# ilovin/lstm_ctc_ocr

Hardware: AMD Instinct MI355X
Metric: captcha images/sec training (32x256, bs=64/GPU) (higher is better)
Workload: dtype bf16; 1 GPU; VGG-7 + BiLSTM(256) + CTC train step, H=32 W=256, 10-char labels, C=64, bs=64/GPU (BASELINE.json configs[1]), Adam lr 1e-4 wd 1e-5 clip 10; global_batch=64, parallelism=dp1, hipgraph=True

## Files before the change

include/ocr_hip.h:

```cpp
#ifndef OCR_HIP_H
#define OCR_HIP_H
#include <stddef.h>
#ifdef __cplusplus
extern "C" {
#endif

enum { OCR_STATUS_OK = 0, OCR_STATUS_MEMOPS = 1, OCR_STATUS_INVALID = 2, OCR_STATUS_EXEC = 3 };

enum {
    OCR_EPI_BIAS = 1, OCR_EPI_RELU = 2, OCR_EPI_OUT_F32 = 4,
    OCR_EPI_MASK = 16, OCR_EPI_ROWSWAP = 32, OCR_EPI_ACCUM = 64
};

const char* ocr_status_string(int status);
int ocr_abi_version(void);
const char* ocr_build_id(void);

int ocr_ctc_workspace_size(int max_label_len, int max_time, int minibatch, size_t* bytes);
int ocr_ctc_loss(const float* activations, float* gradients, const int* flat_labels, const int* label_lengths,
                 const int* input_lengths, int alphabet_size, int minibatch, int max_time, int max_label_len,
                 int blank_label, float* costs, void* workspace, void* stream);
int ocr_ctc_debug(void* dbg);
int ocr_ctc_train_supported(int alphabet_size, int max_time, int max_label_len);
int ocr_ctc_loss_train(const float* activations, void* grad_ntc_bf16, float scale, const int* flat_labels,
// ... 51 lines not shown
                             long strideColsum, void* stream);
typedef struct ocr_tn_job {
    const void* A; long lda; long strideA;
    const void* B; long ldb; long strideB;
    float* out; long ldo; long strideOut;
    float* colsum; long strideColsum;
    int Mk, I, J, nbatch;
    int row_group, row_skip;
    float scale; int reserved;
} ocr_tn_job;
int ocr_gemm_tn_jobs_supported(const ocr_tn_job* jobs, int njobs);
int ocr_gemm_tn_jobs_bf16(const ocr_tn_job* jobs, int njobs, void* stream);
int ocr_set_wgrad_engine(int engine);
int ocr_conv3x3_wgrad_bf16(const void* x, const void* dy, float* dw, float* dbias, int Nb, int W, int H, int Cin,
                           int Cout, int splits, void* stream);
int ocr_conv3x3_wgrad_kernel_choice(int Nb, int W, int H, int Cin, int Cout, int has_workspace, int splits);

int ocr_conv3x3_wgrad_workspace_size(int Nb, int W, int H, int Cin, int Cout, size_t* bytes);
int ocr_conv3x3_wgrad_ws_bf16(const void* x, const void* dy, float* dw, float* dbias, int Nb, int W, int H, int Cin,
                              int Cout, int splits, void* workspace, size_t workspace_bytes, void* stream);
int ocr_conv3x3_wgrad_defer_bf16(const void* x, const void* dy, float* dw, float* dbias, int Nb, int W, int H, int Cin, int Cout,
                                 void* workspace, size_t workspace_bytes, void* job, int* job_blocks, int* deferred, void* stream);
int ocr_wgrad9_reduce_jobs(const void* jobs, int njobs, int total_blocks, void* stream);
int ocr_conv3x3_wgrad_pair_supported(const int* shape_first, const int* shape_second);
int ocr_conv3x3_wgrad_pair_defer_bf16(const void* x0, const void* dy0, float* dw0, float* dbias0, const int* shape0, void* workspace0,
                                      size_t workspace_bytes0, const void* x1, const void* dy1, float* dw1, float* dbias1, const int* shape1,
                                      void* workspace1, size_t workspace_bytes1, void* job0, void* job1, int* job_blocks0, int* job_blocks1,
                                      void* stream);

int ocr_conv1_fwd(const float* x, const float* w, const float* bias, void* y, int Nb, int W, int H, int Cout,
                  int relu, void* stream);
int ocr_conv1_wgrad(const float* x, const void* dz, float* dw, float* db, int Nb, int W, int H, int Cout,
                    void* stream);
int ocr_eltwise_bf16(int op, const void* a, const void* b, void* out, long n, void* stream);
int ocr_conv1_pool_fwd(const float* x, const float* w, const float* bias, void* p, int Nb, int W, int H, int Cout, void* stream);
int ocr_conv1_pool_fwd_train(const float* x, const float* w, const float* bias, void* p, int Nb, int W, int H, int Cout,
                             void* codes, float* zero, long zero_n, void* ones, long ones_n, void* stream);
int ocr_conv1_pool_bwd_codes(const float* x, const float* w, const float* bias, const void* dp, float* dw, float* db,
                             int Nb, int W, int H, int Cout, const void* codes, void* stream);
int ocr_conv1_pool_bwd_slab_rows(int Nb, int W, int H);
int ocr_conv1_pool_bwd_slab(const float* x, const float* w, const float* bias, const void* dp, int Nb, int W, int H, int Cout,
                            const void* codes, float* slab, void* stream);
int ocr_conv1_pool_bwd(const float* x, const float* w, const float* bias, const void* dp, float* dw, float* db, int Nb,
                       int W, int H, int Cout, void* stream);
int ocr_maxpool_fwd(const void* x, void* y, int Nb, int W, int H, int C, int kw, int kh, void* stream);
int ocr_maxpool_bwd(const void* x, const void* dy, void* dx, int Nb, int W, int H, int C, int kw, int kh,
// ... 105 lines not shown
```

lstm_ctc_ocr_amd/_native.py:

```python
import ctypes
import os
import re

_HERE = os.path.dirname(os.path.abspath(__file__))
LIB_PATH = os.environ.get("OCR_NATIVE_LIB") or os.path.join(_HERE, "libocrhip.so")
HEADER_PATH = os.path.join(os.path.dirname(_HERE), "include", "ocr_hip.h")

EPI_BIAS, EPI_RELU, EPI_OUT_F32, EPI_MASK, EPI_ROWSWAP, EPI_ACCUM = 1, 2, 4, 16, 32, 64

_P, _I, _L, _F, _D = ctypes.c_void_p, ctypes.c_int, ctypes.c_long, ctypes.c_float, ctypes.c_double

_SIGS = {
    "ocr_abi_version": ([], _I),
    "ocr_build_id": ([], ctypes.c_char_p),
    "ocr_status_string": ([_I], ctypes.c_char_p),
    "ocr_ctc_workspace_size": ([_I, _I, _I, ctypes.POINTER(ctypes.c_size_t)], _I),
    "ocr_ctc_loss": ([_P, _P, _P, _P, _P, _I, _I, _I, _I, _I, _P, _P, _P], _I),
    "ocr_set_ctc_engine": ([_I], _I),
    "ocr_ctc_debug": ([_P], _I),
    "ocr_ctc_train_supported": ([_I, _I, _I], _I),
    "ocr_ctc_loss_train": ([_P, _P, _F, _P, _P, _P, _I, _I, _I, _I, _I, _P, _P], _I),
    "ocr_ctc_long_placement": ([_I, _I, _I], _I),
    "ocr_ctc_long_supported": ([_I, _I, _I], _I),
    "ocr_ctc_long_workspace_size": ([_I, _I, _I, _I, ctypes.POINTER(ctypes.c_size_t)], _I),
    "ocr_ctc_loss_long": ([_P, _P, _P, _F, _P, _P, _P, _I, _I, _I, _I, _I, _P, _P, ctypes.c_size_t, _P], _I),
    "ocr_ctc_greedy_decode": ([_P, _P, _I, _I, _I, _I, _I, _P, _P, _P], _I),
    "ocr_ctc_beam_workspace_size": ([_I, _I, _I, _I, ctypes.POINTER(ctypes.c_size_t)], _I),
    "ocr_ctc_beam_decode": ([_P, _P, _I, _I, _I, _I, _I, _I, _P, _P, _P, _P, ctypes.c_size_t, _P], _I),
    "ocr_ctc_beam_kernel_choice": ([_I, _I], _I),
    "ocr_set_beam_engine": ([_I], _I),
    "ocr_gemm_nt_bf16": ([_P, _L, _P, _L, _P, _L, _I, _I, _I, _P, _P, _L, _I, _I, _I, _I, _I, _I, _P], _I),
    "ocr_set_gemm_engine": ([_I], _I),
    "ocr_gemm_tn_batched_bf16": ([_P, _L, _L, _P, _L, _L, _P, _L, _L, _I, _I, _I, _I, _F, _I, _P, _L, _P], _I),
    "ocr_gemm_tn_jobs_supported": ([_P, _I], _I),
    "ocr_gemm_tn_jobs_bf16": ([_P, _I, _P], _I),
    "ocr_lstm_xh": ([_P, _P, _P, _P, _I, _I, _I, _I, _I, _P], _I),
    "ocr_set_wgrad_engine": ([_I], _I),
    "ocr_conv3x3_bf16": ([_P, _P, _P, _I, _I, _I, _I, _I, _P, _P, _I, _P], _I),
    "ocr_conv_halo_clock_debug": ([_P], _I),
    "ocr_occupy_cus": ([_I, _I, _I, _F, _P], _I),
    "ocr_conv_ws_debug": ([_P], _I),
    "ocr_conv3x3_accum_supported": ([_I, _I, _I, _I, _I], _I),
    "ocr_conv3x3_kernel_choice": ([_I, _I, _I, _I, _I, _I, _I, _I], _I),
    "ocr_conv3x3_pool_supported": ([_I, _I, _I, _I, _I, _I, _I], _I),
    "ocr_conv3x3_relu_pool_bf16": ([_P, _P, _P, _P, _I, _I, _I, _I, _I, _P, _I, _I, _P], _I),
    "ocr_conv3x3_pool_codes_supported": ([_I, _I, _I, _I, _I, _I, _I], _I),
    "ocr_conv3x3_relu_pool_codes_bf16": ([_P, _P, _P, _P, _P, _I, _I, _I, _I, _I, _P, _I, _I, _P], _I),
    "ocr_gemm_tn_bf16": ([_P, _L, _P, _L, _P, _L, _I, _I, _I, _I, _I, _L, _F, _I, _P, _P], _I),
    "ocr_gemm_tn_split_workspace_floats": ([_I, _I, _I], _L),
    "ocr_gemm_tn_split_bf16": ([_P, _L, _P, _L, _P, _L, _I, _I, _I, _F, _P, _P, _L, _P], _I),
    "ocr_conv3x3_wgrad_bf16": ([_P, _P, _P, _P, _I, _I, _I, _I, _I, _I, _P], _I),
    "ocr_conv3x3_wgrad_kernel_choice": ([_I, _I, _I, _I, _I, _I, _I], _I),
    "ocr_conv3x3_wgrad_workspace_size": ([_I, _I, _I, _I, _I, ctypes.POINTER(ctypes.c_size_t)], _I),
    "ocr_conv3x3_wgrad_ws_bf16": ([_P, _P, _P, _P, _I, _I, _I, _I, _I, _I, _P, ctypes.c_size_t, _P], _I),
    "ocr_conv3x3_wgrad_defer_bf16": ([_P, _P, _P, _P, _I, _I, _I, _I, _I, _P, ctypes.c_size_t, _P, ctypes.POINTER(_I),
                                      ctypes.POINTER(_I), _P], _I),
    "ocr_conv3x3_wgrad_pair_supported": ([ctypes.POINTER(_I), ctypes.POINTER(_I)], _I),
    "ocr_conv3x3_wgrad_pair_defer_bf16": ([_P, _P, _P, _P, ctypes.POINTER(_I), _P, ctypes.c_size_t, _P, _P, _P, _P, ctypes.POINTER(_I), _P,
# ... 68 lines not shown
    "ocr_probe_tr16": ([_P, _P, _P], _I),
    "ocr_set_lstm_proto": ([_I], _I),
    "ocr_set_lstm_ksplit": ([_I], _I),
    "ocr_probe_xcc": ([_P, _I, _I, _P], _I),
    "ocr_mfma_busy_probe": ([_P, _I, _I, _I, _P, _P], _I),
}


class NativeError(RuntimeError):
    pass


def declared_symbols(header=HEADER_PATH):
    text = open(header).read()
    text = re.sub(r"/\*.*?\*/", "", text, flags=re.S)
    return sorted(set(re.findall(r"\b(ocr_[a-z0-9_]+)\s*\(", text)))


def source_build_id(csrc=os.path.join(_HERE, "csrc"), experiments=False):
    import glob
    import hashlib
    rel = [os.path.basename(f) for f in glob.glob(os.path.join(csrc, "*.hip"))]
    h = hashlib.sha256()
    for f in sorted(rel) + ["common.h", "conv_plan.h", "Makefile"]:
        h.update(open(os.path.join(csrc, f), "rb").read())
    return h.hexdigest()[:16] + ("-exp" if experiments else "")


def build_id():
    return lib().ocr_build_id().decode()


_lib = None


def lib():
    global _lib
    if _lib is None:
        if not os.path.exists(LIB_PATH):
            raise NativeError(
                "libocrhip.so not found at %s — build it with `python -c 'import __graft_entry__ as g; g.build()'` "
                "(there is no CPU/eager fallback for the hot path)" % LIB_PATH)
        _lib = ctypes.CDLL(LIB_PATH)
        for name, (argtypes, restype) in _SIGS.items():
            fn = getattr(_lib, name)
            fn.argtypes = argtypes
            fn.restype = restype
# ... 24 lines not shown
```

lstm_ctc_ocr_amd/csrc/gemm_tn3.hip:

```cpp
#include "common.h"
#include <stdlib.h>
#include <type_traits>

struct Tn3Job {
    const bf16_t* A; long lda; long sA;
    const bf16_t* B; long ldb; long sB;
    float* out; long ldo; long sO;
    float* colsum; long sC;
    int Mk, I, J, nbatch;
    int grp, skip;
    float scale; int reserved;
};
static_assert(sizeof(Tn3Job) == 120, "mirrored by lstm_ctc_ocr_amd/ops.py (ctypes.Structure)");

__device__ u32x4 tn3_zero_page[4];

typedef const __attribute__((address_space(1))) void* gptr_t;
typedef __attribute__((address_space(3))) void* lptr_t;
typedef __attribute__((ext_vector_type(4))) short s16x4;
typedef __attribute__((ext_vector_type(8))) short s16x8;

__device__ __forceinline__ int tn3_frag_off(int cb, int lane) {
    const int g = lane >> 4, L = lane & 15;
    const int r0 = 4 * g + (L >> 2);
// ... 186 lines not shown
                old[a2][b][r] = __builtin_nontemporal_load(out + (long)(i0 + wi * 64 + (KH * 2 + a2) * 16 + (lane >> 4) * 4 + r) * g.ldo + j0 + wj * 64 + b * 16 + (lane & 15));
#pragma unroll
    for (int a2 = 0; a2 < 2; ++a2)
#pragma unroll
        for (int b = 0; b < 4; ++b)
#pragma unroll
            for (int r = 0; r < 4; ++r)
                out[(long)(i0 + wi * 64 + (KH * 2 + a2) * 16 + (lane >> 4) * 4 + r) * g.ldo + j0 + wj * 64 + b * 16 + (lane & 15)] =
                    old[a2][b][r] + acc[KH * 2 + a2][b][r] * scale;
}

template <int NST>
__global__ __launch_bounds__(512) __attribute__((amdgpu_waves_per_eu(2, 2))) void gemm_tn3_kernel(Tn3Job j0, Tn3Job j1, int nblk0) {
    extern __shared__ __attribute__((aligned(16))) unsigned char smem[];
    const int kh = __builtin_amdgcn_readfirstlane((int)(threadIdx.x >> 8));
    const int bid = (int)blockIdx.x;
    if (bid < nblk0) {
        if (kh == 0) tn3_body<0, NST>(j0, bid, smem); else tn3_body<1, NST>(j0, bid, smem);
    } else {
        if (kh == 0) tn3_body<0, NST>(j1, bid - nblk0, smem); else tn3_body<1, NST>(j1, bid - nblk0, smem);
    }
}

static bool tn3_covers(const Tn3Job& j) {
    if (!j.A || !j.B || !j.out || j.Mk < 256 || j.I <= 0 || j.J <= 0 || (j.I & 127) || (j.J & 127) || j.nbatch < 1) return false;
    if ((j.lda & 7) || (j.ldb & 7) || (j.sA & 7) || (j.sB & 7) || ((size_t)j.A & 15) || ((size_t)j.B & 15)) return false;
    if (j.grp < 0 || j.skip < 0 || (j.grp == 0 && j.skip != 0)) return false;
    return (long)(j.I >> 7) * (j.J >> 7) * j.nbatch <= 0x7fffffL;
}
extern "C" int ocr_gemm_tn_jobs_supported(const void* jobs, int njobs) {
    if (!jobs || njobs < 1 || njobs > 2) return 0;
    const Tn3Job* j = (const Tn3Job*)jobs;
    for (int k = 0; k < njobs; ++k) if (!tn3_covers(j[k])) return 0;
    return 1;
}
extern "C" int ocr_gemm_tn_jobs_bf16(const void* jobs, int njobs, void* stream) {
    if (!ocr_gemm_tn_jobs_supported(jobs, njobs)) return OCR_ERR_INVALID;
    const Tn3Job* j = (const Tn3Job*)jobs;
    const int t0 = (j[0].I >> 7) * (j[0].J >> 7) * j[0].nbatch;
    const int t1 = njobs > 1 ? (j[1].I >> 7) * (j[1].J >> 7) * j[1].nbatch : 0;
    static int nst = -1;
    if (nst < 0) { const char* e = getenv("OCR_TN3_NST"); nst = (e && atoi(e) == 5) ? 5 : 4; }
    const int lds = nst * 2 * 64 * 256;
    if (nst == 4) {
        if (ocr_allow_lds<gemm_tn3_kernel<4>>(lds) != hipSuccess) return OCR_ERR_EXEC;
        gemm_tn3_kernel<4><<<t0 + t1, 512, lds, (hipStream_t)stream>>>(j[0], njobs > 1 ? j[1] : j[0], t0);
    } else {
        if (ocr_allow_lds<gemm_tn3_kernel<5>>(lds) != hipSuccess) return OCR_ERR_EXEC;
        gemm_tn3_kernel<5><<<t0 + t1, 512, lds, (hipStream_t)stream>>>(j[0], njobs > 1 ? j[1] : j[0], t0);
    }
    OCR_CHECK_LAUNCH();
    return OCR_OK;
}
```

lstm_ctc_ocr_amd/csrc/wgrad9.hip:

```cpp
#include "common.h"
#include <stdlib.h>
#include <utility>
#include <type_traits>

struct W9Args {
    const bf16_t* X; const bf16_t* dY;
    int M, Cin, Cout, cW, cH;
    int k_per_split;
    int S, T_ci, T_co, map;
    float* part;
    float* cs_part;
};

__device__ u32x4 w9_zero_page[4];
typedef const __attribute__((address_space(1))) void* gptr_t;
typedef __attribute__((address_space(3))) void* lptr_t;
typedef __attribute__((ext_vector_type(4))) short s16x4;

constexpr int W9_NDMA = 5;
constexpr int W9_STAGE = 8 * W9_NDMA * 1024;
constexpr int W9_NST = 3;
constexpr int W9_LA = 2;
constexpr int W9_NSLOT = W9_LA + 1;
constexpr int W9_DMA_AT = 3;
// ... 417 lines not shown
    __syncthreads();
    W9P_PHASE(1);

    if (do_cs) w9_cs_store(g, smem, cs, split, co0, tid);
    W9P_PHASE(2);
    w9_store_tile(g, smem, acc, split, ci0, co0, cb, kh, lane);
#ifdef OCR_EXPERIMENTS
    W9P_PHASE(3);
    asm volatile("s_waitcnt vmcnt(0)" ::: "memory");
    W9P_PHASE(4);
#endif
}
template <int H, bool GENW>
__global__ __launch_bounds__(512) void wgrad9p_kernel(W9Args g) { wgrad9p_body<H, GENW>(g, blockIdx.x); }

template <int H, bool GENW>
__global__ __launch_bounds__(512) void wgrad9p_kernel(W9Args first, W9Args second, int nblk_first) {
    const int b = blockIdx.x;
    if (b < nblk_first) wgrad9_body(first, b);
    else if constexpr (H == 16) wgrad9_body(second, b - nblk_first);
    else wgrad9p_body<H, GENW>(second, b - nblk_first);
}

__device__ __forceinline__ void w9_reduce_body(float* __restrict__ dw, const float* __restrict__ part, long n4, long slab4, int S, int rows,
                                               float* __restrict__ dbias, const float* __restrict__ cs_part, int Cout, int blk) {
    __shared__ f32x4 red[256];
    const int cols = 256 / rows;
    const int col = threadIdx.x % cols, row = threadIdx.x / cols;
    const long i = (long)blk * cols + col;
    f32x4 a = {0.f, 0.f, 0.f, 0.f}, t = a;
    if (i < n4) {
        f32x4 b = {0.f, 0.f, 0.f, 0.f}, c = b, d = b;
        const f32x4* p = (const f32x4*)part + i;
        if (row == 0) t = ((const f32x4*)dw)[i];
        int s = row;
        for (; s + 3 * rows < S; s += 4 * rows) {
            a += __builtin_nontemporal_load(p + (long)s * slab4);              b += __builtin_nontemporal_load(p + (long)(s + rows) * slab4);
            c += __builtin_nontemporal_load(p + (long)(s + 2 * rows) * slab4); d += __builtin_nontemporal_load(p + (long)(s + 3 * rows) * slab4);
        }
        for (; s < S; s += rows) a += __builtin_nontemporal_load(p + (long)s * slab4);
        a = (a + b) + (c + d);
    }
    red[row * cols + col] = a;
    __syncthreads();
    if (row == 0 && i < n4) {
        for (int r = 0; r < rows; ++r) t += red[r * cols + col];
        ((f32x4*)dw)[i] = t;
    }
    if (dbias != nullptr && blk == 0)
        for (int c = threadIdx.x; c < Cout; c += blockDim.x) {
            float t = dbias[c];
            for (int s = 0; s < S; ++s) t += cs_part[(long)s * Cout + c];
            dbias[c] = t;
        }
}
__global__ __launch_bounds__(256) void wgrad9_reduce_kernel(float* __restrict__ dw, const float* __restrict__ part, long n4, long slab4,
                                                            int S, int rows, float* __restrict__ dbias, const float* __restrict__ cs_part, int Cout) {
    w9_reduce_body(dw, part, n4, slab4, S, rows, dbias, cs_part, Cout, blockIdx.x);
}
struct W9ReduceJob {
    float* dw; const float* part; float* dbias; const float* cs_part;
    long n4, slab4;
    int S, rows, Cout, block_start;
};
__global__ __launch_bounds__(256) void wgrad9_reduce_jobs_kernel(const W9ReduceJob* __restrict__ jobs, int njobs) {
    __shared__ int jsel[4];
    int j = 0;
    for (int k = threadIdx.x; k < njobs; k += 256)
        if (jobs[k].block_start <= (int)blockIdx.x) j = k;
#pragma unroll
    for (int off = 32; off > 0; off >>= 1) j = max(j, __shfl_xor(j, off));
    if ((threadIdx.x & 63) == 0) jsel[threadIdx.x >> 6] = j;
    __syncthreads();
    j = max(max(jsel[0], jsel[1]), max(jsel[2], jsel[3]));
    const W9ReduceJob jb = jobs[j];
    w9_reduce_body(jb.dw, jb.part, jb.n4, jb.slab4, jb.S, jb.rows, jb.dbias, jb.cs_part, jb.Cout, (int)blockIdx.x - jb.block_start);
}

struct W9Plan { int S, k_per_split, map, T_ci, T_co; size_t bytes; };

static bool w9_plan(int M, int W, int H, int Cin, int Cout, W9Plan* p) {
    if ((Cin & 63) || (Cout & 63) || (H != 2 && H != 4 && H != 8 && H != 16) || M < 512 || (M % H) || W * H < 32) return false;
    const int T_ci = Cin / 64, T_co = Cout / 64, T = T_ci * T_co;
    static int smax = -1;
    if (smax < 0) { const char* e = ocr_tune_env("OCR_W9_SMAX"); smax = e ? atoi(e) : 64; if (smax < 1) smax = 1; }
    int S = 1;
    while ((long)S * 2 * T <= 256 && S * 2 <= smax && M / (S * 2) >= 512) S *= 2;
    p->S = S; p->T_ci = T_ci; p->T_co = T_co;
    p->k_per_split = ceil_div(ceil_div(M, S), 128) * 128;
    p->map = S >= 8 ? 1 : ((T % (8 / S)) == 0 ? 2 : 0);
    p->bytes = (size_t)S * ((size_t)9 * Cin * Cout + Cout) * sizeof(float);
    return true;
}

extern "C" int ocr_wgrad9_debug(void* dbg ) {
    long long* q = (long long*)dbg;
    return hipMemcpyToSymbol(HIP_SYMBOL(w9_dbg), &q, sizeof(q)) == hipSuccess ? OCR_OK : OCR_ERR_MEMOPS;
}

// ... 108 lines not shown
    if (!wgrad9_pair_ok(shape0[0], shape0[1], shape0[2], shape0[3], shape0[4], shape1[0], shape1[1], shape1[2], shape1[3], shape1[4])) return -1;
    W9Plan p0, p1;
    W9Args g0, g1;
    const int k0 = w9_setup(x[0], dy[0], dbias[0], shape0[0], shape0[1], shape0[2], shape0[3], shape0[4], workspace[0], ws_bytes[0], &p0, &g0);
    const int k1 = w9_setup(x[1], dy[1], dbias[1], shape1[0], shape1[1], shape1[2], shape1[3], shape1[4], workspace[1], ws_bytes[1], &p1, &g1);
    if (k0 != W9K_WGRAD9 || k1 < 0) return -1;
    const int grid0 = p0.S * p0.T_ci * p0.T_co, grid1 = p1.S * p1.T_ci * p1.T_co;
    int rc;
    switch (k1) {
        case W9K_P4: rc = w9_launch_pair<W9P_PAIR<4, false>>(g0, grid0, g1, grid1, stream); break;
        case W9K_P8: rc = w9_launch_pair<W9P_PAIR<8, false>>(g0, grid0, g1, grid1, stream); break;
        case W9K_P4_ZERO_ROW: rc = w9_launch_pair<W9P_PAIR<4, true>>(g0, grid0, g1, grid1, stream); break;
        case W9K_P8_ZERO_ROW: rc = w9_launch_pair<W9P_PAIR<8, true>>(g0, grid0, g1, grid1, stream); break;
        default: rc = w9_launch_pair<W9P_PAIR<16, false>>(g0, grid0, g1, grid1, stream); break;
    }
    if (rc != OCR_OK) return rc;
    OCR_CHECK_LAUNCH();
    *(W9ReduceJob*)job[0] = w9_reduce_job(g0, dw[0], dbias[0], job_blocks[0]);
    *(W9ReduceJob*)job[1] = w9_reduce_job(g1, dw[1], dbias[1], job_blocks[1]);
    return OCR_OK;
}

extern "C" int ocr_wgrad9_reduce_jobs(const void* jobs, int njobs, int total_blocks, void* stream) {
    static_assert(sizeof(W9ReduceJob) == 64, "W9ReduceJob is mirrored by engine.py");
    if (!jobs || njobs <= 0 || total_blocks <= 0) return OCR_ERR_INVALID;
    wgrad9_reduce_jobs_kernel<<<total_blocks, 256, 0, (hipStream_t)stream>>>((const W9ReduceJob*)jobs, njobs);
    OCR_CHECK_LAUNCH();
    return OCR_OK;
}
```

lstm_ctc_ocr_amd/engine.py:

```python
import time

import numpy as np
import torch

from . import dist as ocr_dist
from . import ops
from ._native import NativeError, call as nat_call
from .engine_ops import (BF16, F32, I32, _env, _number, _switch, _AddOp, _AvgPoolOp, _BatchNormOp, _BiLstmOp, _ConcatOp, _ConvOp,
                         _Conv3x3Op, _DropoutOp, _FcOp, _InputOp, _PoolOp, _ReluOp, _SoftmaxOp, _SubsampleOp, _ViewOp, _conv_op)
from .layout import FlatLayout, execution_order, init_host_parameters

ALIGN = 64





class ShapePlan(object):

    def _init_fields(self, N, W):
        self.N, self.W = N, W
        self.buf, self.shape = {}, {}
        self.scratch = {}
        self.dy_done = set()
        self.w9_pending, self.w9_tables = [], {}
        self.w9_pending_bytes = 0
        self.tn_pending = []
        self.w9_held = None
        self.tn_side_open = False
        self.fused_pools = set()
        self.bn_stat_rows = {}
        self.bn_bwd_rows = {}
        self.w9_hold_for = {}
        self.unpool_pools = set()
        self.col_bn = {}
        self.lstm_sync_keys = ()
        self.lstm_arena, self.lstm_sync = None, ()
        self.rings_ready, self.rings_armed = set(), False
        self.graph_fb = self.graph_fwd = self.graph_fb1 = self.graph_fb2 = self.graph_dp = self.graph_step = None
        self._guard_addrs = None
        self._report = None

    def __init__(self, eng, N, W):
        self._init_fields(N, W)
        dev = eng.device
        self.x = torch.zeros((N, W, eng.num_features), dtype=F32, device=dev)
        self.labels = torch.zeros(N * eng.max_label_len, dtype=I32, device=dev)
        self.labels_len = torch.zeros(N, dtype=I32, device=dev)
        self.seq_len = torch.ones(N, dtype=I32, device=dev)
        self.oshape = {'data': (N, W, eng.num_features)}
# ... 31 lines not shown
class Engine(object):

    def __init__(self, net, device='cuda:0', seed=None, max_label_len=31, use_graphs=True, group=None,
                 persistent_lstm=True, fuse_conv1_pool=True, ctc_long=True):
        from .config import cfg
        if max_label_len > self.CTC_MAX_LABEL_LEN:
            raise ValueError('max_label_len = %d: the CTC loss covers labels of at most %d characters' % (max_label_len, self.CTC_MAX_LABEL_LEN))
        if not torch.cuda.is_available():
            raise NativeError('Engine needs a ROCm GPU: the hot path has no CPU implementation')
        self.cfg = cfg
        self.net = net
        self.device = torch.device(device)
        torch.cuda.set_device(self.device)
        self.num_features = cfg.NUM_FEATURES
        self.max_label_len = max_label_len
        self.ctc_long = ctc_long
        self.use_graphs = use_graphs
        self.persistent_lstm = persistent_lstm
        self.fuse_conv1_pool = fuse_conv1_pool
        self.fuse_bn_stats = _switch('OCR_FUSE_BN_STATS')
        self.w9_flush_bytes = int(_number('OCR_W9_FLUSH_MB', 80, float) * (1 << 20))
        self.tn_defer = _switch('OCR_TN_JOBS')
        self.tn_side = _switch('OCR_TN_SIDE', False)
        self.side_stream = torch.cuda.Stream(device=self.device) if (self.tn_side and torch.device(self.device).type == 'cuda') else None
        self.group = group
        self.world = 1
        self._check_xcd_placement()
        self.force_allreduce = bool(_env('OCR_FORCE_ALLREDUCE'))
        if group is not None or (torch.distributed.is_available() and torch.distributed.is_initialized()):
            self.world = torch.distributed.get_world_size(group)
        if _env('OCR_FAKE_WORLD'):
            self.world = _number('OCR_FAKE_WORLD', None)
            self.force_allreduce = True
        self.overlap_allreduce = _switch('OCR_OVERLAP_ALLREDUCE')
        self.dp_graph = _env('OCR_DP_GRAPH', '0') == '1'
        self.defer_w9 = _switch('OCR_W9_DEFER')
        self.w9_pair = _switch('OCR_W9_PAIR')
        self.w9_defer_max_bytes = _number('OCR_W9_DEFER_MAX_MB', self.W9_DEFER_MAX_BYTES >> 20) << 20
        self.w9_ws_pool = {}
        self.comm_stream = torch.cuda.Stream(device=self.device)
        self.dp_host_s = [0.0, 0.0, 0.0, 0.0, 0.0, 0]
        self._pack_table = None
        self._fault_hook = None
        self._watch_pending = None
        self.dropped_reports = 0
        self._lower(net)
# ... 267 lines not shown
            d.copy_(t, non_blocking=True)

    def step_counter(self):
        return self.scalars[6:7]

    def _forward(self, sp, training=False):
        self.training = training
        self._zero_pending = bool(training) and self.grads.numel() % 4 == 0 and _switch('OCR_FUSE_ZERO')
        if training and not self._zero_pending:
            self.grads.zero_()
        sp.rings_ready, sp.rings_armed = set(), False
        self._ones_pending = sp.lstm_arena if (training and sp.lstm_arena is not None and _switch('OCR_FUSE_RINGFILL')) else None
        for op in self.ops:
            op.fwd(sp)
        self._ones_pending = None
        if self._zero_pending:
            self.grads.zero_()
            self._zero_pending = False

    def _loss_and_backward(self, sp, flush=True):
        sp.dy_done = set()
        sp.w9_pending = []
        sp.tn_pending = []
        sp.w9_held = None
        logits = self.ops[-1].y(sp)
        scale = ocr_dist.loss_scale(sp.N, self.world)
        path = self.ctc_path_of(sp.C, sp.T)
        if path == 'fast':
            ops.ctc_loss_train(logits, self.ops[-1].dy(sp), scale, sp.labels, sp.labels_len, sp.seq_len, self.max_label_len,
                               sp.costs, blank=0)
        elif path == 'long':
            ops.ctc_loss_long(logits, sp.labels, sp.labels_len, sp.seq_len, self.max_label_len, blank=0, want_grad=False,
                              grad_ntc_bf16=self.ops[-1].dy(sp), scale=scale, workspace=sp.ctc_ws, costs=sp.costs)
        else:
            ops.ctc_loss(logits, sp.labels, sp.labels_len, sp.seq_len, self.max_label_len, blank=0, want_grad=True,
                         workspace=sp.ctc_ws, costs=sp.costs, grads=sp.ctc_grad)
            ops.tnc_to_ntc_bf16(sp.ctc_grad, self.ops[-1].dy(sp), scale)
        for op in reversed(self.ops[self.split_op:]):
            op.bwd(sp)
        self._flush_tn(sp)
        self._join_tn(sp)
        self._release_w9(sp)
        if flush:
            self._flush_w9(sp)

    CTC_MAX_LABEL_LEN = 255

    def ctc_path_of(self, C, T):
        if ops.ctc_train_supported(C, T, self.max_label_len):
            return 'fast'
        if self.ctc_long and ops.ctc_long_supported(C, T, self.max_label_len):
            return 'long'
        return 'general'

    def ctc_path(self, N, W):
        sp = self.plan(N, W)
        return self.ctc_path_of(sp.C, sp.T)

    def _backward_early(self, sp):
        for op in reversed(self.ops[:self.split_op]):
            op.bwd(sp)
        self._flush_tn(sp)
        self._join_tn(sp)
        self._release_w9(sp)
        self._flush_w9(sp)

    def tn_push(self, sp, job, keep, fallback):
        if not self.tn_defer or not ops.gemm_tn_jobs_supported([job]):
            fallback()
            return
        sp.tn_pending.append((job, keep, fallback))
        if len(sp.tn_pending) == 2:
            self._flush_tn(sp)

    def _flush_tn(self, sp):
        pend, sp.tn_pending = sp.tn_pending, []
        if len(pend) == 2:
            if self.tn_side:
                main = torch.cuda.current_stream(self.device)
                self.side_stream.wait_stream(main)
                with torch.cuda.stream(self.side_stream):
                    ops.gemm_tn_jobs([pend[0][0], pend[1][0]])
                sp.tn_side_open = True
            else:
                ops.gemm_tn_jobs([pend[0][0], pend[1][0]])
        else:
            for _, _, fallback in pend:
                fallback()

    def _join_tn(self, sp):
        if sp.tn_side_open:
            torch.cuda.current_stream(self.device).wait_stream(self.side_stream)
            sp.tn_side_open = False

    W9_DEFER_MAX_BYTES = 192 << 20
    W9_JOB_DTYPE = np.dtype([('dw', '<u8'), ('part', '<u8'), ('dbias', '<u8'), ('cs_part', '<u8'), ('n4', '<i8'), ('slab4', '<i8'),
                             ('S', '<i4'), ('rows', '<i4'), ('Cout', '<i4'), ('block_start', '<i4')])

    def w9_append(self, sp, job, ws):
        sp.w9_pending.append(job)
        sp.w9_pending_bytes += ws.numel()
        if self.w9_flush_bytes and sp.w9_pending_bytes >= self.w9_flush_bytes:
            self._flush_w9(sp)

    def w9_hold(self, sp, key, x, dz, dw, db, ws):
        self._release_w9(sp)
        sp.w9_held = (key, x, dz, dw, db, ws)

    def _release_w9(self, sp):
        held, sp.w9_held = sp.w9_held, None
        if held is not None:
            _, x, dz, dw, db, ws = held
            job, nblk = ops.conv3x3_wgrad_deferred(x, dz, dw, db, ws)
            if job is not None:
                self.w9_append(sp, (job, nblk), ws)

    def _flush_w9(self, sp):
        self._release_w9(sp)
        pend, sp.w9_pending = sp.w9_pending, []
        sp.w9_pending_bytes = 0
        if not pend:
            return
        raw = b''.join(job for job, _ in pend)
        ent = sp.w9_tables.get(raw)
        if ent is None:
            tab = np.frombuffer(raw, dtype=self.W9_JOB_DTYPE).copy()
            assert tab.itemsize == 64 and len(tab) == len(pend)
            start = 0
            for i, (_, nblk) in enumerate(pend):
                tab['block_start'][i] = start
                start += nblk
            dev = torch.from_numpy(tab.view(np.uint8).copy()).to(self.device)
            ent = sp.w9_tables[raw] = (dev, len(pend), start)
        ops.wgrad9_reduce_jobs(*ent)

    def _capture(self, fn):
        import gc
        gc.collect()
        torch.cuda.synchronize()
        g = torch.cuda.CUDAGraph()
        was = gc.isenabled()
        gc.disable()
        try:
            with torch.cuda.graph(g, capture_error_mode='thread_local'):
                fn()
        finally:
            if was:
                gc.enable()
        return g

    def _run_split(self, sp):
        def body1():
            self._forward(sp, training=True)
            self._loss_and_backward(sp)
            self._publish_guard(sp)

        def body2():
# ... 319 lines not shown
```

lstm_ctc_ocr_amd/ops.py:

```python
import ctypes

import torch

from . import _native as nat
from ._native import EPI_ACCUM, EPI_BIAS, EPI_MASK, EPI_OUT_F32, EPI_RELU, EPI_ROWSWAP, call, ptr

BF16 = torch.bfloat16
F32 = torch.float32


def _st():
    return nat.stream()


def _dev(t):
    if not t.is_cuda:
        raise nat.NativeError("hot-path operators take device tensors only (got a CPU tensor)")
    return t


def ctc_workspace_bytes(max_label_len, max_time, minibatch):
    sz = ctypes.c_size_t(0)
    call("ocr_ctc_workspace_size", max_label_len, max_time, minibatch, ctypes.byref(sz))
    return sz.value
# ... 218 lines not shown
                ("B", ctypes.c_void_p), ("ldb", ctypes.c_long), ("strideB", ctypes.c_long),
                ("out", ctypes.c_void_p), ("ldo", ctypes.c_long), ("strideOut", ctypes.c_long),
                ("colsum", ctypes.c_void_p), ("strideColsum", ctypes.c_long),
                ("Mk", ctypes.c_int), ("I", ctypes.c_int), ("J", ctypes.c_int), ("nbatch", ctypes.c_int),
                ("row_group", ctypes.c_int), ("row_skip", ctypes.c_int), ("scale", ctypes.c_float), ("reserved", ctypes.c_int)]


def tn_job(A, lda, B, ldb, out, ldo, Mk, I, J, *, nbatch=1, strideA=0, strideB=0, strideOut=0, colsum=None, strideColsum=0, row_group=0,
           row_skip=0, scale=1.0):
    return TnJob(ptr(_dev(A)), lda, strideA, ptr(_dev(B)), ldb, strideB, ptr(out), ldo, strideOut, ptr(colsum), strideColsum,
                 Mk, I, J, nbatch, row_group, row_skip, float(scale), 0)


def gemm_tn_jobs_supported(jobs):
    arr = (TnJob * len(jobs))(*jobs)
    return bool(nat.lib().ocr_gemm_tn_jobs_supported(ctypes.cast(arr, ctypes.c_void_p), len(jobs)))


def gemm_tn_jobs(jobs):
    arr = (TnJob * len(jobs))(*jobs)
    call("ocr_gemm_tn_jobs_bf16", ctypes.cast(arr, ctypes.c_void_p), len(jobs), _st())


def lstm_xh(x2d, hout, seq_len, xh, Nb, T, D, U, ndir=2):
    call("ocr_lstm_xh", ptr(_dev(x2d)), ptr(hout), ptr(seq_len), ptr(xh), Nb, T, D, U, ndir, _st())
    return xh


def conv3x3_wgrad_workspace_bytes(Nb, W, H, Cin, Cout):
    sz = ctypes.c_size_t(0)
    call("ocr_conv3x3_wgrad_workspace_size", Nb, W, H, Cin, Cout, ctypes.byref(sz))
    return sz.value


WGRAD_KERNEL_NAMES = ("wgrad9", "wgrad9p<4>", "wgrad9p<8>", "wgrad9p<4>/zero-row", "wgrad9p<8>/zero-row", "gemm_tn2/nine-tap",
                      "gemm_tn2/paired-tap", "gemm_tn<1,4,4>", "gemm_tn<1,2,2>")


def conv3x3_wgrad_kernel_choice(Nb, W, H, Cin, Cout, *, workspace=True, splits=0):
    rc = nat.lib().ocr_conv3x3_wgrad_kernel_choice(int(Nb), int(W), int(H), int(Cin), int(Cout), int(bool(workspace)), int(splits))
    if rc < 0:
        raise nat.NativeError("ocr_conv3x3_wgrad_kernel_choice failed: status %d (%s)" % (-rc, nat.status_string(-rc)))
    return WGRAD_KERNEL_NAMES[rc & 255], rc >> 8


def conv3x3_wgrad(x, dy, dw, splits=0, dbias=None, workspace=None):
# ... 404 lines not shown
```

Baseline: 58120 images/sec.

## Fuse deferred TN weight-grad GEMM pair with wgrad9 split-K reduction launch

Holds the pending pair of TN weight-gradient GEMM jobs and, when the wgrad9 split-K reduce jobs are flushed, launches both in one kernel. The GEMM blocks come first and the tail blocks run the reduction as two virtual 256-thread blocks per 512-thread block, sharing LDS. This aims to remove one launch and the tail or idle gap between the GEMM and the small reduce kernel. The cost is that the reduce blocks now run at the GEMM kernel's LDS allocation and occupancy, and the held GEMM work may be delayed to the flush point, which changes the ordering.

```diff
diff --git a/include/ocr_hip.h b/include/ocr_hip.h
--- a/include/ocr_hip.h
+++ b/include/ocr_hip.h
@@ -97,6 +97,9 @@
 int ocr_conv3x3_wgrad_defer_bf16(const void* x, const void* dy, float* dw, float* dbias, int Nb, int W, int H, int Cin, int Cout,
                                  void* workspace, size_t workspace_bytes, void* job, int* job_blocks, int* deferred, void* stream);
 int ocr_wgrad9_reduce_jobs(const void* jobs, int njobs, int total_blocks, void* stream);
+int ocr_gemm_tn_jobs_reduce_supported(const ocr_tn_job* jobs, int njobs, const void* reduce_jobs, int n_reduce_jobs, int total_reduce_blocks);
+int ocr_gemm_tn_jobs_reduce_bf16(const ocr_tn_job* jobs, int njobs, const void* reduce_jobs, int n_reduce_jobs, int total_reduce_blocks,
+                                 void* stream);
 int ocr_conv3x3_wgrad_pair_supported(const int* shape_first, const int* shape_second);
 int ocr_conv3x3_wgrad_pair_defer_bf16(const void* x0, const void* dy0, float* dw0, float* dbias0, const int* shape0, void* workspace0,
                                       size_t workspace_bytes0, const void* x1, const void* dy1, float* dw1, float* dbias1, const int* shape1,
diff --git a/lstm_ctc_ocr_amd/_native.py b/lstm_ctc_ocr_amd/_native.py
--- a/lstm_ctc_ocr_amd/_native.py
+++ b/lstm_ctc_ocr_amd/_native.py
@@ -34,6 +34,8 @@
     "ocr_gemm_tn_batched_bf16": ([_P, _L, _L, _P, _L, _L, _P, _L, _L, _I, _I, _I, _I, _F, _I, _P, _L, _P], _I),
     "ocr_gemm_tn_jobs_supported": ([_P, _I], _I),
     "ocr_gemm_tn_jobs_bf16": ([_P, _I, _P], _I),
+    "ocr_gemm_tn_jobs_reduce_supported": ([_P, _I, _P, _I, _I], _I),
+    "ocr_gemm_tn_jobs_reduce_bf16": ([_P, _I, _P, _I, _I, _P], _I),
     "ocr_lstm_xh": ([_P, _P, _P, _P, _I, _I, _I, _I, _I, _P], _I),
     "ocr_set_wgrad_engine": ([_I], _I),
     "ocr_conv3x3_bf16": ([_P, _P, _P, _I, _I, _I, _I, _I, _P, _P, _I, _P], _I),
@@ -148,7 +150,7 @@
     import hashlib
     rel = [os.path.basename(f) for f in glob.glob(os.path.join(csrc, "*.hip"))]
     h = hashlib.sha256()
-    for f in sorted(rel) + ["common.h", "conv_plan.h", "Makefile"]:
+    for f in sorted(rel) + ["common.h", "conv_plan.h", "w9_reduce.h", "Makefile"]:
         h.update(open(os.path.join(csrc, f), "rb").read())
     return h.hexdigest()[:16] + ("-exp" if experiments else "")
 
diff --git a/lstm_ctc_ocr_amd/csrc/gemm_tn3.hip b/lstm_ctc_ocr_amd/csrc/gemm_tn3.hip
--- a/lstm_ctc_ocr_amd/csrc/gemm_tn3.hip
+++ b/lstm_ctc_ocr_amd/csrc/gemm_tn3.hip
@@ -1,4 +1,5 @@
 #include "common.h"
+#include "w9_reduce.h"
 #include <stdlib.h>
 #include <type_traits>
 
@@ -232,6 +233,26 @@
     }
 }
 
+template <int NST>
+__global__ __launch_bounds__(512) __attribute__((amdgpu_waves_per_eu(2, 2))) void gemm_tn3_kernel(Tn3Job j0, Tn3Job j1, int nblk0, int nblk_tn,
+                                                                                              const W9ReduceJob* __restrict__ jobs, int njobs, int nvirt) {
+    extern __shared__ __attribute__((aligned(16))) unsigned char smem[];
+    const int kh = __builtin_amdgcn_readfirstlane((int)(threadIdx.x >> 8));
+    const int bid = (int)blockIdx.x;
+    if (bid < nblk0) {
+        if (kh == 0) tn3_body<0, NST>(j0, bid, smem); else tn3_body<1, NST>(j0, bid, smem);
+    } else if (bid < nblk_tn) {
+        if (kh == 0) tn3_body<0, NST>(j1, bid - nblk0, smem); else tn3_body<1, NST>(j1, bid - nblk0, smem);
+    } else {
+        const int vblk = 2 * (bid - nblk_tn) + kh, tid = (int)threadIdx.x & (W9R_THREADS - 1);
+        f32x4* red = (f32x4*)(smem + kh * W9R_RED_BYTES);
+        int* jsel = (int*)(smem + 2 * W9R_RED_BYTES + kh * W9R_JSEL_BYTES);
+        const int j = w9_reduce_find_job(jobs, njobs, vblk, tid, jsel);
+        const W9ReduceJob jb = jobs[j];
+        w9_reduce_body(jb.dw, jb.part, jb.n4, jb.slab4, jb.S, jb.rows, jb.dbias, jb.cs_part, jb.Cout, vblk - jb.block_start, tid, red, vblk < nvirt);
+    }
+}
+
 static bool tn3_covers(const Tn3Job& j) {
     if (!j.A || !j.B || !j.out || j.Mk < 256 || j.I <= 0 || j.J <= 0 || (j.I & 127) || (j.J & 127) || j.nbatch < 1) return false;
     if ((j.lda & 7) || (j.ldb & 7) || (j.sA & 7) || (j.sB & 7) || ((size_t)j.A & 15) || ((size_t)j.B & 15)) return false;
@@ -244,21 +265,60 @@
     for (int k = 0; k < njobs; ++k) if (!tn3_covers(j[k])) return 0;
     return 1;
 }
+typedef void (*Tn3Kernel)(Tn3Job, Tn3Job, int);
+typedef void (*Tn3ReduceKernel)(Tn3Job, Tn3Job, int, int, const W9ReduceJob*, int, int);
+template <int NST> constexpr Tn3Kernel TN3_PLAIN = gemm_tn3_kernel<NST>;
+template <int NST> constexpr Tn3ReduceKernel TN3_REDUCE = gemm_tn3_kernel<NST>;
+
+static int tn3_stages() {
+    static int nst = -1;
+    if (nst < 0) { const char* e = getenv("OCR_TN3_NST"); nst = (e && atoi(e) == 5) ? 5 : 4; }
+    return nst;
+}
+static int tn3_tiles(const Tn3Job& j) { return (j.I >> 7) * (j.J >> 7) * j.nbatch; }
+
 extern "C" int ocr_gemm_tn_jobs_bf16(const void* jobs, int njobs, void* stream) {
     if (!ocr_gemm_tn_jobs_supported(jobs, njobs)) return OCR_ERR_INVALID;
     const Tn3Job* j = (const Tn3Job*)jobs;
-    const int t0 = (j[0].I >> 7) * (j[0].J >> 7) * j[0].nbatch;
-    const int t1 = njobs > 1 ? (j[1].I >> 7) * (j[1].J >> 7) * j[1].nbatch : 0;
-    static int nst = -1;
-    if (nst < 0) { const char* e = getenv("OCR_TN3_NST"); nst = (e && atoi(e) == 5) ? 5 : 4; }
+    const int t0 = tn3_tiles(j[0]);
+    const int t1 = njobs > 1 ? tn3_tiles(j[1]) : 0;
+    const int nst = tn3_stages();
     const int lds = nst * 2 * 64 * 256;
     if (nst == 4) {
-        if (ocr_allow_lds<gemm_tn3_kernel<4>>(lds) != hipSuccess) return OCR_ERR_EXEC;
-        gemm_tn3_kernel<4><<<t0 + t1, 512, lds, (hipStream_t)stream>>>(j[0], njobs > 1 ? j[1] : j[0], t0);
+        if (ocr_allow_lds<TN3_PLAIN<4>>(lds) != hipSuccess) return OCR_ERR_EXEC;
+        TN3_PLAIN<4><<<t0 + t1, 512, lds, (hipStream_t)stream>>>(j[0], njobs > 1 ? j[1] : j[0], t0);
     } else {
-        if (ocr_allow_lds<gemm_tn3_kernel<5>>(lds) != hipSuccess) return OCR_ERR_EXEC;
-        gemm_tn3_kernel<5><<<t0 + t1, 512, lds, (hipStream_t)stream>>>(j[0], njobs > 1 ? j[1] : j[0], t0);
+        if (ocr_allow_lds<TN3_PLAIN<5>>(lds) != hipSuccess) return OCR_ERR_EXEC;
+        TN3_PLAIN<5><<<t0 + t1, 512, lds, (hipStream_t)stream>>>(j[0], njobs > 1 ? j[1] : j[0], t0);
     }
     OCR_CHECK_LAUNCH();
     return OCR_OK;
 }
+
+extern "C" int ocr_gemm_tn_jobs_reduce_supported(const void* jobs, int njobs, const void* reduce_jobs, int n_reduce_jobs, int total_reduce_blocks) {
+    if (!ocr_gemm_tn_jobs_supported(jobs, njobs)) return 0;
+    if (!reduce_jobs || n_reduce_jobs < 1 || total_reduce_blocks < 1) return 0;
+    const Tn3Job* j = (const Tn3Job*)jobs;
+    return (long)tn3_tiles(j[0]) + (njobs > 1 ? tn3_tiles(j[1]) : 0) + ((long)total_reduce_blocks + 1) / 2 <= 0x7fffffffL;
+}
+extern "C" int ocr_gemm_tn_jobs_reduce_bf16(const void* jobs, int njobs, const void* reduce_jobs, int n_reduce_jobs, int total_reduce_blocks,
+                                            void* stream) {
+    if (!ocr_gemm_tn_jobs_reduce_supported(jobs, njobs, reduce_jobs, n_reduce_jobs, total_reduce_blocks)) return OCR_ERR_INVALID;
+    const Tn3Job* j = (const Tn3Job*)jobs;
+    const int t0 = tn3_tiles(j[0]);
+    const int t1 = njobs > 1 ? tn3_tiles(j[1]) : 0;
+    const int grid = t0 + t1 + (total_reduce_blocks + 1) / 2;
+    const int nst = tn3_stages();
+    const int lds = nst * 2 * 64 * 256;
+    static_assert(2 * (W9R_RED_BYTES + W9R_JSEL_BYTES) <= 2 * 64 * 256, "the virtual blocks' LDS fits one stage");
+    const W9ReduceJob* rj = (const W9ReduceJob*)reduce_jobs;
+    if (nst == 4) {
+        if (ocr_allow_lds<TN3_REDUCE<4>>(lds) != hipSuccess) return OCR_ERR_EXEC;
+        TN3_REDUCE<4><<<grid, 512, lds, (hipStream_t)stream>>>(j[0], njobs > 1 ? j[1] : j[0], t0, t0 + t1, rj, n_reduce_jobs, total_reduce_blocks);
+    } else {
+        if (ocr_allow_lds<TN3_REDUCE<5>>(lds) != hipSuccess) return OCR_ERR_EXEC;
+        TN3_REDUCE<5><<<grid, 512, lds, (hipStream_t)stream>>>(j[0], njobs > 1 ? j[1] : j[0], t0, t0 + t1, rj, n_reduce_jobs, total_reduce_blocks);
+    }
+    OCR_CHECK_LAUNCH();
+    return OCR_OK;
+}
diff --git a/lstm_ctc_ocr_amd/csrc/w9_reduce.h b/lstm_ctc_ocr_amd/csrc/w9_reduce.h
--- /dev/null
+++ b/lstm_ctc_ocr_amd/csrc/w9_reduce.h
@@ -0,0 +1,57 @@
+#pragma once
+#include "common.h"
+
+struct W9ReduceJob {
+    float* dw; const float* part; float* dbias; const float* cs_part;
+    long n4, slab4;
+    int S, rows, Cout, block_start;
+};
+static_assert(sizeof(W9ReduceJob) == 64, "W9ReduceJob is mirrored by engine.py");
+
+constexpr int W9R_THREADS = 256;
+constexpr int W9R_RED_BYTES = W9R_THREADS * 16;
+constexpr int W9R_JSEL_BYTES = 16;
+
+__device__ __forceinline__ void w9_reduce_body(float* __restrict__ dw, const float* __restrict__ part, long n4, long slab4, int S, int rows,
+                                               float* __restrict__ dbias, const float* __restrict__ cs_part, int Cout, int blk, int tid,
+                                               f32x4* red, bool live) {
+    const int cols = W9R_THREADS / rows;
+    const int col = tid % cols, row = tid / cols;
+    const long i = (long)blk * cols + col;
+    f32x4 a = {0.f, 0.f, 0.f, 0.f}, t = a;
+    if (live && i < n4) {
+        f32x4 b = {0.f, 0.f, 0.f, 0.f}, c = b, d = b;
+        const f32x4* p = (const f32x4*)part + i;
+        if (row == 0) t = ((const f32x4*)dw)[i];
+        int s = row;
+        for (; s + 3 * rows < S; s += 4 * rows) {
+            a += __builtin_nontemporal_load(p + (long)s * slab4);              b += __builtin_nontemporal_load(p + (long)(s + rows) * slab4);
+            c += __builtin_nontemporal_load(p + (long)(s + 2 * rows) * slab4); d += __builtin_nontemporal_load(p + (long)(s + 3 * rows) * slab4);
+        }
+        for (; s < S; s += rows) a += __builtin_nontemporal_load(p + (long)s * slab4);
+        a = (a + b) + (c + d);
+    }
+    red[row * cols + col] = a;
+    __syncthreads();
+    if (live && row == 0 && i < n4) {
+        for (int r = 0; r < rows; ++r) t += red[r * cols + col];
+        ((f32x4*)dw)[i] = t;
+    }
+    if (live && dbias != nullptr && blk == 0)
+        for (int c = tid; c < Cout; c += W9R_THREADS) {
+            float t = dbias[c];
+            for (int s = 0; s < S; ++s) t += cs_part[(long)s * Cout + c];
+            dbias[c] = t;
+        }
+}
+
+__device__ __forceinline__ int w9_reduce_find_job(const W9ReduceJob* __restrict__ jobs, int njobs, int vblk, int tid, int* jsel) {
+    int j = 0;
+    for (int k = tid; k < njobs; k += W9R_THREADS)
+        if (jobs[k].block_start <= vblk) j = k;
+#pragma unroll
+    for (int off = 32; off > 0; off >>= 1) j = max(j, __shfl_xor(j, off));
+    if ((tid & 63) == 0) jsel[tid >> 6] = j;
+    __syncthreads();
+    return max(max(jsel[0], jsel[1]), max(jsel[2], jsel[3]));
+}
diff --git a/lstm_ctc_ocr_amd/csrc/wgrad9.hip b/lstm_ctc_ocr_amd/csrc/wgrad9.hip
--- a/lstm_ctc_ocr_amd/csrc/wgrad9.hip
+++ b/lstm_ctc_ocr_amd/csrc/wgrad9.hip
@@ -1,4 +1,5 @@
 #include "common.h"
+#include "w9_reduce.h"
 #include <stdlib.h>
 #include <utility>
 #include <type_traits>
@@ -463,59 +464,17 @@
     else wgrad9p_body<H, GENW>(second, b - nblk_first);
 }
 
-__device__ __forceinline__ void w9_reduce_body(float* __restrict__ dw, const float* __restrict__ part, long n4, long slab4, int S, int rows,
-                                               float* __restrict__ dbias, const float* __restrict__ cs_part, int Cout, int blk) {
-    __shared__ f32x4 red[256];
-    const int cols = 256 / rows;
-    const int col = threadIdx.x % cols, row = threadIdx.x / cols;
-    const long i = (long)blk * cols + col;
-    f32x4 a = {0.f, 0.f, 0.f, 0.f}, t = a;
-    if (i < n4) {
-        f32x4 b = {0.f, 0.f, 0.f, 0.f}, c = b, d = b;
-        const f32x4* p = (const f32x4*)part + i;
-        if (row == 0) t = ((const f32x4*)dw)[i];
-        int s = row;
-        for (; s + 3 * rows < S; s += 4 * rows) {
-            a += __builtin_nontemporal_load(p + (long)s * slab4);              b += __builtin_nontemporal_load(p + (long)(s + rows) * slab4);
-            c += __builtin_nontemporal_load(p + (long)(s + 2 * rows) * slab4); d += __builtin_nontemporal_load(p + (long)(s + 3 * rows) * slab4);
-        }
-        for (; s < S; s += rows) a += __builtin_nontemporal_load(p + (long)s * slab4);
-        a = (a + b) + (c + d);
-    }
-    red[row * cols + col] = a;
-    __syncthreads();
-    if (row == 0 && i < n4) {
-        for (int r = 0; r < rows; ++r) t += red[r * cols + col];
-        ((f32x4*)dw)[i] = t;
-    }
-    if (dbias != nullptr && blk == 0)
-        for (int c = threadIdx.x; c < Cout; c += blockDim.x) {
-            float t = dbias[c];
-            for (int s = 0; s < S; ++s) t += cs_part[(long)s * Cout + c];
-            dbias[c] = t;
-        }
-}
 __global__ __launch_bounds__(256) void wgrad9_reduce_kernel(float* __restrict__ dw, const float* __restrict__ part, long n4, long slab4,
                                                             int S, int rows, float* __restrict__ dbias, const float* __restrict__ cs_part, int Cout) {
-    w9_reduce_body(dw, part, n4, slab4, S, rows, dbias, cs_part, Cout, blockIdx.x);
-}
-struct W9ReduceJob {
-    float* dw; const float* part; float* dbias; const float* cs_part;
-    long n4, slab4;
-    int S, rows, Cout, block_start;
-};
+    __shared__ f32x4 red[W9R_THREADS];
+    w9_reduce_body(dw, part, n4, slab4, S, rows, dbias, cs_part, Cout, blockIdx.x, threadIdx.x, red, true);
+}
 __global__ __launch_bounds__(256) void wgrad9_reduce_jobs_kernel(const W9ReduceJob* __restrict__ jobs, int njobs) {
+    __shared__ f32x4 red[W9R_THREADS];
     __shared__ int jsel[4];
-    int j = 0;
-    for (int k = threadIdx.x; k < njobs; k += 256)
-        if (jobs[k].block_start <= (int)blockIdx.x) j = k;
-#pragma unroll
-    for (int off = 32; off > 0; off >>= 1) j = max(j, __shfl_xor(j, off));
-    if ((threadIdx.x & 63) == 0) jsel[threadIdx.x >> 6] = j;
-    __syncthreads();
-    j = max(max(jsel[0], jsel[1]), max(jsel[2], jsel[3]));
+    const int j = w9_reduce_find_job(jobs, njobs, (int)blockIdx.x, threadIdx.x, jsel);
     const W9ReduceJob jb = jobs[j];
-    w9_reduce_body(jb.dw, jb.part, jb.n4, jb.slab4, jb.S, jb.rows, jb.dbias, jb.cs_part, jb.Cout, (int)blockIdx.x - jb.block_start);
+    w9_reduce_body(jb.dw, jb.part, jb.n4, jb.slab4, jb.S, jb.rows, jb.dbias, jb.cs_part, jb.Cout, (int)blockIdx.x - jb.block_start, threadIdx.x, red, true);
 }
 
 struct W9Plan { int S, k_per_split, map, T_ci, T_co; size_t bytes; };
@@ -670,7 +629,6 @@
 }
 
 extern "C" int ocr_wgrad9_reduce_jobs(const void* jobs, int njobs, int total_blocks, void* stream) {
-    static_assert(sizeof(W9ReduceJob) == 64, "W9ReduceJob is mirrored by engine.py");
     if (!jobs || njobs <= 0 || total_blocks <= 0) return OCR_ERR_INVALID;
     wgrad9_reduce_jobs_kernel<<<total_blocks, 256, 0, (hipStream_t)stream>>>((const W9ReduceJob*)jobs, njobs);
     OCR_CHECK_LAUNCH();
diff --git a/lstm_ctc_ocr_amd/engine.py b/lstm_ctc_ocr_amd/engine.py
--- a/lstm_ctc_ocr_amd/engine.py
+++ b/lstm_ctc_ocr_amd/engine.py
@@ -11,6 +11,7 @@
 from .layout import FlatLayout, execution_order, init_host_parameters
 
 ALIGN = 64
+TN_REDUCE_DEFAULT = True
 
 
 
@@ -26,6 +27,7 @@
         self.w9_pending, self.w9_tables = [], {}
         self.w9_pending_bytes = 0
         self.tn_pending = []
+        self.tn_held = None
         self.w9_held = None
         self.tn_side_open = False
         self.fused_pools = set()
@@ -103,6 +105,7 @@
         self.w9_flush_bytes = int(_number('OCR_W9_FLUSH_MB', 80, float) * (1 << 20))
         self.tn_defer = _switch('OCR_TN_JOBS')
         self.tn_side = _switch('OCR_TN_SIDE', False)
+        self.tn_reduce = self.tn_reduce_enabled(self.tn_defer, self.tn_side)
         self.side_stream = torch.cuda.Stream(device=self.device) if (self.tn_side and torch.device(self.device).type == 'cuda') else None
         self.group = group
         self.world = 1
@@ -416,6 +419,7 @@
         sp.dy_done = set()
         sp.w9_pending = []
         sp.tn_pending = []
+        sp.tn_held = None
         sp.w9_held = None
         logits = self.ops[-1].y(sp)
         scale = ocr_dist.loss_scale(sp.N, self.world)
@@ -437,6 +441,7 @@
         self._release_w9(sp)
         if flush:
             self._flush_w9(sp)
+            self._release_tn(sp)
 
     CTC_MAX_LABEL_LEN = 255
 
@@ -458,6 +463,11 @@
         self._join_tn(sp)
         self._release_w9(sp)
         self._flush_w9(sp)
+        self._release_tn(sp)
+
+    @staticmethod
+    def tn_reduce_enabled(tn_defer, tn_side):
+        return bool(_switch('OCR_TN_REDUCE', TN_REDUCE_DEFAULT) and tn_defer and not tn_side)
 
     def tn_push(self, sp, job, keep, fallback):
         if not self.tn_defer or not ops.gemm_tn_jobs_supported([job]):
@@ -476,11 +486,19 @@
                 with torch.cuda.stream(self.side_stream):
                     ops.gemm_tn_jobs([pend[0][0], pend[1][0]])
                 sp.tn_side_open = True
+            elif self.tn_reduce:
+                self._release_tn(sp)
+                sp.tn_held = pend
             else:
                 ops.gemm_tn_jobs([pend[0][0], pend[1][0]])
         else:
             for _, _, fallback in pend:
                 fallback()
+
+    def _release_tn(self, sp):
+        held, sp.tn_held = sp.tn_held, None
+        if held is not None:
+            ops.gemm_tn_jobs([held[0][0], held[1][0]])
 
     def _join_tn(self, sp):
         if sp.tn_side_open:
@@ -526,7 +544,11 @@
                 start += nblk
             dev = torch.from_numpy(tab.view(np.uint8).copy()).to(self.device)
             ent = sp.w9_tables[raw] = (dev, len(pend), start)
-        ops.wgrad9_reduce_jobs(*ent)
+        held, sp.tn_held = sp.tn_held, None
+        if held is not None:
+            ops.gemm_tn_jobs_reduce([held[0][0], held[1][0]], *ent)
+        else:
+            ops.wgrad9_reduce_jobs(*ent)
 
     def _capture(self, fn):
         import gc
diff --git a/lstm_ctc_ocr_amd/ops.py b/lstm_ctc_ocr_amd/ops.py
--- a/lstm_ctc_ocr_amd/ops.py
+++ b/lstm_ctc_ocr_amd/ops.py
@@ -264,6 +264,16 @@
     call("ocr_gemm_tn_jobs_bf16", ctypes.cast(arr, ctypes.c_void_p), len(jobs), _st())
 
 
+def gemm_tn_jobs_reduce_supported(jobs, table, njobs, total_blocks):
+    arr = (TnJob * len(jobs))(*jobs)
+    return bool(nat.lib().ocr_gemm_tn_jobs_reduce_supported(ctypes.cast(arr, ctypes.c_void_p), len(jobs), ptr(table), njobs, total_blocks))
+
+
+def gemm_tn_jobs_reduce(jobs, table, njobs, total_blocks):
+    arr = (TnJob * len(jobs))(*jobs)
+    call("ocr_gemm_tn_jobs_reduce_bf16", ctypes.cast(arr, ctypes.c_void_p), len(jobs), ptr(table if table is None else _dev(table)), njobs, total_blocks, _st())
+
+
 def lstm_xh(x2d, hout, seq_len, xh, Nb, T, D, U, ndir=2):
     call("ocr_lstm_xh", ptr(_dev(x2d)), ptr(hout), ptr(seq_len), ptr(xh), Nb, T, D, U, ndir, _st())
     return xh
```

After: 58680 images/sec, median of 6. About the same (+1.0%).
